# TonyLianLong/LLM-groundedDiffusion

Hardware: AMD Instinct MI355X
Metric: images/sec (50-step SD1.5 512^2, LMD+ guidance) (higher is better)
Workload: dtype fp16; 1 GPU; LMD+ stage 2, 4 cached 2-box layouts/GPU/step (lmd_v0.1 cache), 50 DDIM steps, 512x512, sd14_gligen (SD1.4+GLIGEN architecture, seeded random weights), VAE decodes included; per-box masks = box masks; mask_refinement=box, layouts_per_gpu=4, num_inference_steps=50, parallelism=dp1, rccl_ranks=1, lanes_per_gpu=4, gemm_tuning=throughput

## Files before the change

### llm-groundeddiffusion_amd/build.py

```python
import hashlib
import os
import subprocess
import sys

HERE = os.path.dirname(os.path.abspath(__file__))
CSRC = os.path.join(HERE, "csrc")
OUT = os.path.join(HERE, "liblgd_hip.so")
STAMP = OUT + ".stamp"
SOURCES = ["gemm.hip", "norm.hip", "attn.hip", "attn_w4.hip", "attn_bwd.hip", "misc.hip", "energy.hip", "boxdiff.hip", "sam.hip", "options.hip", "detect.hip", "sam_tail.hip", "handoff.hip"]
FLAGS = ["--offload-arch=gfx950", "-O3", "-std=c++17", "-fPIC",
         "-Wno-unused-value"]
EXTRA_FLAGS = {"attn.hip": ["-mllvm", "-amdgpu-mfma-vgpr-form=1"],
               "attn_bwd.hip": ["-mllvm", "-amdgpu-mfma-vgpr-form=1"],
               "sam_tail.hip": ["-ffp-contract=off"],
               "handoff.hip": ["-ffp-contract=off"]}


def _digest():
    h = hashlib.sha256()
    files = [os.path.join(CSRC, f) for f in sorted(os.listdir(CSRC))]
    files.append(os.path.join(HERE, "..", "include", "lgd_hip.h"))
    for f in files:
        with open(f, "rb") as fh:
            h.update(fh.read())
    h.update(" ".join(FLAGS).encode())
    h.update(repr(sorted(EXTRA_FLAGS.items())).encode())
    return h.hexdigest()


def build(force=False, verbose=True):
    dig = _digest()
    if not force and os.path.exists(OUT) and os.path.exists(STAMP):
        if open(STAMP).read().strip() == dig:
            return OUT
    hipcc = os.environ.get("HIPCC", "/opt/rocm/bin/hipcc")
    objs = []
    procs = []
    os.makedirs(os.path.join(HERE, "build"), exist_ok=True)
    for s in SOURCES:
        o = os.path.join(HERE, "build", s.replace(".hip", ".o"))
        cmd = [hipcc] + FLAGS + EXTRA_FLAGS.get(s, []) + ["-c", os.path.join(CSRC, s), "-o", o]
        procs.append((s, subprocess.Popen(cmd, stdout=subprocess.PIPE, stderr=subprocess.STDOUT)))
        objs.append(o)
    for s, p in procs:
        out, _ = p.communicate()
        if p.returncode != 0:
            raise RuntimeError(f"hipcc failed on {s}:\n{out.decode()}")
        if verbose and out.strip():
            print(out.decode())
    cmd = [hipcc, "--offload-arch=gfx950", "-shared", "-fPIC", "-o", OUT] + objs
    r = subprocess.run(cmd, stdout=subprocess.PIPE, stderr=subprocess.STDOUT)
    if r.returncode != 0:
        raise RuntimeError(f"link failed:\n{r.stdout.decode()}")
    with open(STAMP, "w") as fh:
        fh.write(dig)
    if verbose:
        print(f"built {OUT}")
    return OUT


if __name__ == "__main__":
    build(force="--force" in sys.argv)
```

### llm-groundeddiffusion_amd/csrc/attn_bwd.hip

```cpp
#include "common.h"
#include "../../include/lgd_hip.h"
#include "attn_plan.h"
#include <stdlib.h>

namespace {

constexpr int T64 = 64;
constexpr int TR_LD = T64 + 8;

template <int DP, int NT = 256>
struct PairTile {
  static constexpr int KSEG = DP / 8;
  static constexpr int ITEMS = (T64 / 2) * KSEG;
  static constexpr int IT = (ITEMS + NT - 1) / NT;
  uint4 v[IT][2];

  __device__ __forceinline__ void load(const half_t* __restrict__ src, long ld, int row0, int nrows, int d) {
#pragma unroll
    for (int i = 0; i < IT; ++i) {
      const int idx = threadIdx.x + i * NT;
      const int pair = idx & 31, seg = idx >> 5;
#pragma unroll
      for (int r = 0; r < 2; ++r) {
        const int row = row0 + pair * 2 + r;
        const bool ok = idx < ITEMS && row < nrows && seg * 8 < d;
        v[i][r] = ok ? *reinterpret_cast<const uint4*>(src + (long)row * ld + seg * 8) : make_uint4(0, 0, 0, 0);
      }
    }
  }
  template <bool RM, bool TR>
  __device__ __forceinline__ void store(half_t* rm, half_t* tr) const {
#pragma unroll
    for (int i = 0; i < IT; ++i) {
      const int idx = threadIdx.x + i * NT;
      if (idx >= ITEMS) continue;
      const int pair = idx & 31, seg = idx >> 5;
      if (RM) {
        *reinterpret_cast<uint4*>(rm + (pair * 2) * (DP + 16) + seg * 8) = v[i][0];
        *reinterpret_cast<uint4*>(rm + (pair * 2 + 1) * (DP + 16) + seg * 8) = v[i][1];
      }
      if (TR) {
        const uint32_t w0[4] = {v[i][0].x, v[i][0].y, v[i][0].z, v[i][0].w};
        const uint32_t w1[4] = {v[i][1].x, v[i][1].y, v[i][1].z, v[i][1].w};
#pragma unroll
        for (int j = 0; j < 4; ++j) {
          const uint32_t even = (w0[j] & 0xffffu) | (w1[j] << 16);
          const uint32_t odd = (w0[j] >> 16) | (w1[j] & 0xffff0000u);
          *reinterpret_cast<uint32_t*>(tr + (seg * 8 + 2 * j) * TR_LD + pair * 2) = even;
          *reinterpret_cast<uint32_t*>(tr + (seg * 8 + 2 * j + 1) * TR_LD + pair * 2) = odd;
        }
      }
    }
  }
};

struct AttnBwdArgs {
  const half_t* q; long ldq, q_bs;
  const half_t* k; long ldk, k_bs;
  const half_t* v; long ldv, v_bs;
  const half_t* o; long ldo, o_bs;
  const half_t* go; long ldgo, go_bs;
  const float* lse;
  float* delta;
  half_t* gq; long ldgq, gq_bs;
  half_t* gk; long ldgk, gk_bs;
  half_t* gv; long ldgv, gv_bs;
  int B, H, Sq, Sk, d;
  int sk_grad;
  float scale, scale_log2;
};

__device__ __forceinline__ half8_t tr_frag(const half_t* tr, int row, int c, int g) {
  const half_t* p = tr + row * TR_LD + c * 32 + g * 4;
  half4_t lo = *reinterpret_cast<const half4_t*>(p);
  half4_t hi = *reinterpret_cast<const half4_t*>(p + 16);
  return (half8_t){lo[0], lo[1], lo[2], lo[3], hi[0], hi[1], hi[2], hi[3]};
}

template <int DP, int QT, int NDT, int NW = 4, bool DB = false>
__global__ __launch_bounds__(64 * NW) void attn_bwd_dq_kernel(const AttnBwdArgs a) {
  constexpr int K_LD = DP + 16;
  constexpr int NDC = DP / 32;
  constexpr int STAGE = 2 * T64 * K_LD + DP * TR_LD;
  extern __shared__ __attribute__((aligned(16))) char dyn_smem[];
  half_t* const smem = reinterpret_cast<half_t*>(dyn_smem);
  half_t* Ks = smem;
  half_t* Vs = Ks + T64 * K_LD;
  half_t* Kt = Vs + T64 * K_LD;

  const int tid = threadIdx.x, lane = tid & 63, wid = tid >> 6;
  const int g = lane >> 4, c16 = lane & 15;
  const int b = blockIdx.z, h = blockIdx.y;
  const int d = a.d;
  const int q0 = blockIdx.x * (16 * NW * QT) + wid * (16 * QT);
  const half_t* Qb = a.q + (long)b * a.q_bs + (long)h * d;
  const half_t* Kb = a.k + (long)b * a.k_bs + (long)h * d;
  const half_t* Vb = a.v + (long)b * a.v_bs + (long)h * d;
  const half_t* Ob = a.o + (long)b * a.o_bs + (long)h * d;
  const half_t* GOb = a.go + (long)b * a.go_bs + (long)h * d;

  half8_t qf[QT][NDC], dof[QT][NDC];
  float delta[QT], nlse[QT];
#pragma unroll
  for (int qt = 0; qt < QT; ++qt) {
    const int qrow = q0 + qt * 16 + c16;
    const bool q_ok = qrow < a.Sq;
    float dl = 0.f;
#pragma unroll
    for (int dc = 0; dc < NDC; ++dc) {
      const int dd = dc * 32 + g * 8;
      if (q_ok && dd < d) {
        qf[qt][dc] = *reinterpret_cast<const half8_t*>(Qb + (long)qrow * a.ldq + dd);
        dof[qt][dc] = *reinterpret_cast<const half8_t*>(GOb + (long)qrow * a.ldgo + dd);
        half8_t of = *reinterpret_cast<const half8_t*>(Ob + (long)qrow * a.ldo + dd);
#pragma unroll
        for (int e = 0; e < 8; ++e) dl += (float)dof[qt][dc][e] * (float)of[e];
      } else {
        qf[qt][dc] = (half8_t){0, 0, 0, 0, 0, 0, 0, 0};
        dof[qt][dc] = (half8_t){0, 0, 0, 0, 0, 0, 0, 0};
      }
    }
    dl += __shfl_xor(dl, 16, 64);
    dl += __shfl_xor(dl, 32, 64);
    const long stat_idx = ((long)b * a.H + h) * a.Sq + qrow;
    if (q_ok && g == 0) a.delta[stat_idx] = dl;
    delta[qt] = dl;
    nlse[qt] = q_ok ? -a.lse[stat_idx] : 0.f;
  }

  f32x4 dq[QT][NDT];
#pragma unroll
  for (int qt = 0; qt < QT; ++qt)
#pragma unroll
    for (int dt = 0; dt < NDT; ++dt) dq[qt][dt] = (f32x4){0.f, 0.f, 0.f, 0.f};

  const float sl2 = a.scale_log2;
  const int n_tiles = (a.Sk + T64 - 1) / T64;
  PairTile<DP, 64 * NW> kreg, vreg;
  kreg.load(Kb, a.ldk, 0, a.Sk, d);
  vreg.load(Vb, a.ldv, 0, a.Sk, d);
  kreg.template store<true, true>(Ks, Kt);
  vreg.template store<true, false>(Vs, nullptr);
  __syncthreads();
  for (int t = 0; t < n_tiles; ++t) {
    const int kv0 = t * T64;
    if constexpr (DB) {
      Ks = smem + (t & 1) * STAGE;
      Vs = Ks + T64 * K_LD;
      Kt = Vs + T64 * K_LD;
    }
    if (t + 1 < n_tiles) {
      kreg.load(Kb, a.ldk, kv0 + T64, a.Sk, d);
      vreg.load(Vb, a.ldv, kv0 + T64, a.Sk, d);
    }
    f32x4 ds[QT][4];
#pragma unroll
    for (int kt = 0; kt < 4; ++kt) {
      half8_t kf[NDC], vf[NDC];
#pragma unroll
      for (int dc = 0; dc < NDC; ++dc) {
        kf[dc] = *reinterpret_cast<const half8_t*>(Ks + (kt * 16 + c16) * K_LD + dc * 32 + g * 8);
        vf[dc] = *reinterpret_cast<const half8_t*>(Vs + (kt * 16 + c16) * K_LD + dc * 32 + g * 8);
      }
#pragma unroll
      for (int qt = 0; qt < QT; ++qt) {
        f32x4 sv = {0.f, 0.f, 0.f, 0.f}, dp = {0.f, 0.f, 0.f, 0.f};
#pragma unroll
        for (int dc = 0; dc < NDC; ++dc) {
          sv = __builtin_amdgcn_mfma_f32_16x16x32_f16(kf[dc], qf[qt][dc], sv, 0, 0, 0);
          dp = __builtin_amdgcn_mfma_f32_16x16x32_f16(vf[dc], dof[qt][dc], dp, 0, 0, 0);
        }
#pragma unroll
        for (int r = 0; r < 4; ++r) {
          const float pv = __builtin_amdgcn_exp2f(fmaf(sv[r], sl2, nlse[qt]));
          ds[qt][kt][r] = pv * (dp[r] - delta[qt]);
        }
      }
    }
    if (kv0 + T64 > a.Sk) {
#pragma unroll
      for (int qt = 0; qt < QT; ++qt)
#pragma unroll
        for (int kt = 0; kt < 4; ++kt)
#pragma unroll
          for (int r = 0; r < 4; ++r)
            if (kv0 + kt * 16 + g * 4 + r >= a.Sk) ds[qt][kt][r] = 0.f;
    }
#pragma unroll
    for (int c = 0; c < 2; ++c) {
      half8_t dsf[QT];
#pragma unroll
      for (int qt = 0; qt < QT; ++qt)
#pragma unroll
        for (int r = 0; r < 4; ++r) {
          dsf[qt][r] = (half_t)ds[qt][2 * c][r];
          dsf[qt][4 + r] = (half_t)ds[qt][2 * c + 1][r];
        }
#pragma unroll
      for (int dt = 0; dt < NDT; ++dt) {
        half8_t ktf = tr_frag(Kt, dt * 16 + c16, c, g);
#pragma unroll
        for (int qt = 0; qt < QT; ++qt)
          dq[qt][dt] = __builtin_amdgcn_mfma_f32_16x16x32_f16(ktf, dsf[qt], dq[qt][dt], 0, 0, 0);
      }
    }
    if constexpr (DB) {
      if (t + 1 < n_tiles) {
        half_t* nK = smem + ((t + 1) & 1) * STAGE;
        kreg.template store<true, true>(nK, nK + 2 * T64 * K_LD);
        vreg.template store<true, false>(nK + T64 * K_LD, nullptr);
      }
      __syncthreads();
    } else {
      __syncthreads();
      if (t + 1 < n_tiles) {
        kreg.template store<true, true>(Ks, Kt);
        vreg.template store<true, false>(Vs, nullptr);
        __syncthreads();
      }
    }
  }
#pragma unroll
// ... 319 lines not shown
  const half_t* Vb = a.v + (long)b * a.v_bs + (long)h * d;

  for (int idx = tid; idx < XM_KEYS * KSEG; idx += 256) {
    const int row = idx / KSEG, seg = idx - row * KSEG;
    const bool ok = row < Sk && seg * 8 < d;
    const uint4 kk = ok ? *reinterpret_cast<const uint4*>(Kb + (long)row * a.ldk + seg * 8) : make_uint4(0, 0, 0, 0);
    const uint4 vv = ok ? *reinterpret_cast<const uint4*>(Vb + (long)row * a.ldv + seg * 8) : make_uint4(0, 0, 0, 0);
    *reinterpret_cast<uint4*>(Ks + row * K_LD + seg * 8) = kk;
    *reinterpret_cast<uint4*>(Vs + row * K_LD + seg * 8) = vv;
    const half_t* e = reinterpret_cast<const half_t*>(&kk);
#pragma unroll
    for (int j = 0; j < 8; ++j) Kt[(seg * 8 + j) * XM_LD + row] = e[j];
  }
  __syncthreads();

  const float sl2 = a.scale * 1.4426950408889634f;
  const int q_blk = blockIdx.x * 256;
  for (int it = 0; it < 4; ++it) {
    const int qrow = q_blk + it * 64 + wid * 16 + c16;
    if (q_blk + it * 64 + wid * 16 >= a.Sq) break;
    const bool q_ok = qrow < a.Sq;
    half8_t qf[NDC], gof[NDC];
#pragma unroll
    for (int dc = 0; dc < NDC; ++dc) {
      const int dd = dc * 32 + g * 8;
      qf[dc] = (half8_t){0, 0, 0, 0, 0, 0, 0, 0};
      gof[dc] = qf[dc];
      if (q_ok && dd < d) {
        qf[dc] = *reinterpret_cast<const half8_t*>(a.q + (long)b * a.q_bs + (long)qrow * a.ldq + (long)h * d + dd);
        if (a.go)
          gof[dc] = *reinterpret_cast<const half8_t*>(a.go + (long)b * a.go_bs + (long)qrow * a.ldgo + (long)h * d + dd);
      }
    }
    f32x4 sv[NKT], dp[NKT];
#pragma unroll
    for (int kt = 0; kt < NKT; ++kt) {
      f32x4 s = {0.f, 0.f, 0.f, 0.f}, t = {0.f, 0.f, 0.f, 0.f};
#pragma unroll
      for (int dc = 0; dc < NDC; ++dc) {
        half8_t kf = *reinterpret_cast<const half8_t*>(Ks + (kt * 16 + c16) * K_LD + dc * 32 + g * 8);
        half8_t vf = *reinterpret_cast<const half8_t*>(Vs + (kt * 16 + c16) * K_LD + dc * 32 + g * 8);
        s = __builtin_amdgcn_mfma_f32_16x16x32_f16(kf, qf[dc], s, 0, 0, 0);
        t = __builtin_amdgcn_mfma_f32_16x16x32_f16(vf, gof[dc], t, 0, 0, 0);
      }
      sv[kt] = s;
      dp[kt] = t;
    }
    float mx = -1.0e30f;
#pragma unroll
    for (int kt = 0; kt < NKT; ++kt)
#pragma unroll
      for (int r = 0; r < 4; ++r) {
        if (kt * 16 + g * 4 + r >= Sk) sv[kt][r] = -1.0e30f;
        mx = fmaxf(mx, sv[kt][r]);
      }
    mx = fmaxf(mx, __shfl_xor(mx, 16, 64));
    mx = fmaxf(mx, __shfl_xor(mx, 32, 64));
    const float nm = -mx * sl2;
    float sum = 0.f;
#pragma unroll
    for (int kt = 0; kt < NKT; ++kt)
#pragma unroll
      for (int r = 0; r < 4; ++r) {
        const float p = __builtin_amdgcn_exp2f(fmaf(sv[kt][r], sl2, nm));
        sv[kt][r] = p;
        sum += p;
      }
    sum += __shfl_xor(sum, 16, 64);
    sum += __shfl_xor(sum, 32, 64);
    const float inv = 1.f / sum;
    if (a.gp && q_ok) {
      const float* gpr = a.gp + (((long)b * a.H + h) * a.Sq + qrow) * Sk;
#pragma unroll
      for (int kt = 0; kt < NKT; ++kt)
#pragma unroll
        for (int r = 0; r < 4; ++r) {
          const int key = kt * 16 + g * 4 + r;
          if (key < Sk) dp[kt][r] += gpr[key];
        }
    }
    float dot = 0.f;
#pragma unroll
    for (int kt = 0; kt < NKT; ++kt)
#pragma unroll
      for (int r = 0; r < 4; ++r) {
        sv[kt][r] *= inv;
        dot += sv[kt][r] * dp[kt][r];
      }
    dot += __shfl_xor(dot, 16, 64);
    dot += __shfl_xor(dot, 32, 64);
    f32x4 dq[NDT];
#pragma unroll
    for (int dt = 0; dt < NDT; ++dt) dq[dt] = (f32x4){0.f, 0.f, 0.f, 0.f};
#pragma unroll
    for (int c = 0; c < NKT / 2; ++c) {
      half8_t dsf;
#pragma unroll
      for (int r = 0; r < 4; ++r) {
        dsf[r] = (half_t)(sv[2 * c][r] * (dp[2 * c][r] - dot) * a.scale);
        dsf[4 + r] = (half_t)(sv[2 * c + 1][r] * (dp[2 * c + 1][r] - dot) * a.scale);
      }
#pragma unroll
      for (int dt = 0; dt < NDT; ++dt) {
        const half_t* pk = Kt + (dt * 16 + c16) * XM_LD + c * 32 + g * 4;
        half4_t lo = *reinterpret_cast<const half4_t*>(pk);
        half4_t hi = *reinterpret_cast<const half4_t*>(pk + 16);
        half8_t ktf = {lo[0], lo[1], lo[2], lo[3], hi[0], hi[1], hi[2], hi[3]};
        dq[dt] = __builtin_amdgcn_mfma_f32_16x16x32_f16(ktf, dsf, dq[dt], 0, 0, 0);
      }
    }
    if (q_ok) {
      half_t* out = a.gq + (long)b * a.gq_bs + (long)qrow * a.ldgq + (long)h * d;
#pragma unroll
      for (int dt = 0; dt < NDT; ++dt) {
        const int dv = dt * 16 + g * 4;
        if (dv < d) {
          half4_t o;
#pragma unroll
          for (int r = 0; r < 4; ++r) o[r] = (half_t)dq[dt][r];
          *reinterpret_cast<half4_t*>(out + dv) = o;
        }
      }
    }
  }
}

template <int DP>
int launch_cross_bwd_mfma(const CrossBwdArgs& a, hipStream_t st) {
  const size_t smem = (size_t)(2 * XM_KEYS * (DP + 16) + DP * XM_LD) * 2;
  static const bool attr_set = [smem] {
    (void)hipFuncSetAttribute(reinterpret_cast<const void*>(&cross_attn_bwd_mfma_kernel<DP>),
                              hipFuncAttributeMaxDynamicSharedMemorySize, (int)smem);
    return true;
  }();
  (void)attr_set;
  hipLaunchKernelGGL((cross_attn_bwd_mfma_kernel<DP>), dim3((a.Sq + 255) / 256, a.H, a.B), dim3(256), smem, st, a);
  return lgd_check_launch();
}

int launch_cross_bwd_rows(const CrossBwdArgs& a, hipStream_t st) {
  const int ld = a.d + 2;
  size_t smem = (size_t)(2 * a.Sk * ld + 2) * 2 + (size_t)4 * 2 * XB_MAXD * 4 + (size_t)4 * XB_MAXSK * 4;
  smem = (smem + 15) & ~(size_t)15;
  static const bool attr_set = [] {
    (void)hipFuncSetAttribute(reinterpret_cast<const void*>(&cross_attn_bwd_kernel),
                        hipFuncAttributeMaxDynamicSharedMemorySize, 160 * 1024);
    return true;
  }();
  (void)attr_set;
  hipLaunchKernelGGL(cross_attn_bwd_kernel, dim3((a.Sq + 4 * XB_ROWS - 1) / (4 * XB_ROWS), a.H, a.B), dim3(256), smem, st, a);
  return lgd_check_launch();
}

template <int DP, int THREE, int SHAPE>
int launch_bwd(const AttnBwdArgs& a, hipStream_t st) {
  static_assert(!THREE || DP == 64, "the three-tile form is the d = 40 head at DP = 64");
  constexpr int NT = SHAPE == BWD_T1 ? 1 : 2, NDT = THREE ? 3 : DP / 16, NW = SHAPE == BWD_T2_DB_NW8 ? 8 : 4;
  constexpr bool DB = SHAPE == BWD_T2_DB || SHAPE == BWD_T2_DB_NW8;
  constexpr int K_LD = DP + 16;
  constexpr int NST = DB ? 2 : 1;
  const size_t smem_dq = (size_t)NST * (2 * T64 * K_LD + DP * TR_LD) * 2;
  const size_t smem_dkv = (size_t)NST * ((2 * T64 * K_LD + 2 * DP * TR_LD) * 2 + 2 * T64 * 4);
  static const bool attr_set = [smem_dq, smem_dkv] {
    (void)hipFuncSetAttribute(reinterpret_cast<const void*>(&attn_bwd_dkv_kernel<DP, NT, NDT, NW, DB>),
                        hipFuncAttributeMaxDynamicSharedMemorySize, (int)smem_dkv);
    (void)hipFuncSetAttribute(reinterpret_cast<const void*>(&attn_bwd_dq_kernel<DP, NT, NDT, NW, DB>),
                        hipFuncAttributeMaxDynamicSharedMemorySize, (int)smem_dq);
    return true;
  }();
  (void)attr_set;
  hipLaunchKernelGGL((attn_bwd_dq_kernel<DP, NT, NDT, NW, DB>), dim3((a.Sq + 16 * NW * NT - 1) / (16 * NW * NT), a.H, a.B),
                     dim3(64 * NW), smem_dq, st, a);
  hipLaunchKernelGGL((attn_bwd_dkv_kernel<DP, NT, NDT, NW, DB>), dim3((a.sk_grad + 16 * NW * NT - 1) / (16 * NW * NT), a.H, a.B),
                     dim3(64 * NW), smem_dkv, st, a);
  return lgd_check_launch();
}

int attn_bwd_env() {
  static const int env = [] { const char* e = getenv("LGD_ATTN_BWD"); return e ? atoi(e) : -2; }();
  return env;
}

int bwd_dp_of(int d) { return d <= 32 ? 32 : d <= 64 ? 64 : d <= 96 ? 96 : d <= 128 ? 128 : d <= 160 ? 160 : 0; }

int plan_bwd(int B, int H, int Sq, int Sk, int d) {
  const int DP = bwd_dp_of(d);
  if (!DP) return LGD_ERR_UNSUPPORTED;
  const long wgs = (long)((Sq < Sk ? Sq : Sk) / 128) * H * B;
  const int env = attn_bwd_env();
  const bool narrow = env == -2;
  const int mode = narrow ? 0 : env;
  if (DP == 64 && d <= 48) {
    if (wgs < 512) return attn_code(ATTN_FAM_BWD, DP, 10 + BWD_T1);
    if ((narrow || mode == 2) && wgs >= 1024) return attn_code(ATTN_FAM_BWD, DP, 10 + BWD_T2_DB_NW8);
    if (narrow || mode >= 1) return attn_code(ATTN_FAM_BWD, DP, 10 + BWD_T2_DB);
    return attn_code(ATTN_FAM_BWD, DP, 10 + BWD_T2);
  }
  if (DP <= 96 && wgs >= 512) {
    if (DP == 64 && mode == 2 && wgs >= 1024) return attn_code(ATTN_FAM_BWD, DP, BWD_T2_DB_NW8);
    if (mode >= 1) return attn_code(ATTN_FAM_BWD, DP, BWD_T2_DB);
    return attn_code(ATTN_FAM_BWD, DP, BWD_T2);
  }
  return attn_code(ATTN_FAM_BWD, DP, BWD_T1);
}

int plan_cross_bwd(int Sk, int d, bool aligned) {
  if (Sk < 1 || Sk > XB_MAXSK || d > XB_MAXD) return LGD_ERR_ARG;
  if (Sk <= XM_KEYS && d <= 160 && aligned) return attn_code(ATTN_FAM_XBWD_MFMA, bwd_dp_of(d), 0);
  return attn_code(ATTN_FAM_XBWD_ROWS, 0, 0);
}

#define BWD_NAME_T1 "1 tile per wave"
#define BWD_NAME_T2 "2 tiles per wave"
#define BWD_NAME_T2_DB "2 tiles per wave, double-buffered"
#define BWD_NAME_T2_DB_NW8 "2 tiles per wave, double-buffered, 8 waves"
#define BWD_NAME_THREE_0 " "
#define BWD_NAME_THREE_1 " (d <= 48, 3 tiles of d) "
#define BWD_ROW(DP, THREE, SHAPE, ENV)                                                                              \
  {{attn_code(ATTN_FAM_BWD, DP, 10 * THREE + BWD_##SHAPE), ENV,                                                     \
    "attn_bwd_dq/dkv_kernel DP=" #DP BWD_NAME_THREE_##THREE BWD_NAME_##SHAPE},                                      \
   launch_bwd<DP, THREE, BWD_##SHAPE>}
#define XBWD_MFMA_ROW(DP) {{attn_code(ATTN_FAM_XBWD_MFMA, DP, 0), 0, "cross_attn_bwd_mfma_kernel DP=" #DP}, launch_cross_bwd_mfma<DP>}

const AttnVariant<AttnBwdArgs> BWD_VARIANTS[] = {
    BWD_ROW(32, 0, T1, 0), BWD_ROW(32, 0, T2, 0), BWD_ROW(32, 0, T2_DB, 1),
    BWD_ROW(64, 0, T1, 0), BWD_ROW(64, 0, T2, 0), BWD_ROW(64, 0, T2_DB, 1), BWD_ROW(64, 0, T2_DB_NW8, 1),
    BWD_ROW(64, 1, T1, 0), BWD_ROW(64, 1, T2, 1), BWD_ROW(64, 1, T2_DB, 0), BWD_ROW(64, 1, T2_DB_NW8, 0),
    BWD_ROW(96, 0, T1, 0), BWD_ROW(96, 0, T2, 0), BWD_ROW(96, 0, T2_DB, 1),
    BWD_ROW(128, 0, T1, 0), BWD_ROW(160, 0, T1, 0),
};
const AttnVariant<CrossBwdArgs> XBWD_VARIANTS[] = {
    XBWD_MFMA_ROW(32), XBWD_MFMA_ROW(64), XBWD_MFMA_ROW(96), XBWD_MFMA_ROW(128), XBWD_MFMA_ROW(160),
    {{attn_code(ATTN_FAM_XBWD_ROWS, 0, 0), 0, "cross_attn_bwd_kernel (one wave per query row)"}, launch_cross_bwd_rows},
};
constexpr int N_BWD_VARIANTS = sizeof(BWD_VARIANTS) / sizeof(BWD_VARIANTS[0]);
constexpr int N_XBWD_VARIANTS = sizeof(XBWD_VARIANTS) / sizeof(XBWD_VARIANTS[0]);
static_assert(N_BWD_VARIANTS == 16 && N_XBWD_VARIANTS == 5 + 1, "a kernel instantiation was added or dropped");

}

int lgd_attn_bwd_plan(int B, int H, int Sq, int Sk, int d) { return plan_bwd(B, H, Sq, Sk, d); }
int lgd_cross_attn_bwd_plan(int Sk, int d, int aligned) { return plan_cross_bwd(Sk, d, aligned != 0); }
const AttnVariantInfo* lgd_attn_bwd_variant_info(int index) {
  if (index < 0) return nullptr;
  if (index < N_BWD_VARIANTS) return &BWD_VARIANTS[index].info;
  index -= N_BWD_VARIANTS;
  return index < N_XBWD_VARIANTS ? &XBWD_VARIANTS[index].info : nullptr;
}

extern "C" int lgd_attn_bwd_keys_f16(const void* q, int64_t ldq, int64_t q_bs, const void* k,
                                     int64_t ldk, int64_t k_bs, const void* v, int64_t ldv, int64_t v_bs,
                                     const void* o, int64_t ldo, int64_t o_bs, const void* go,
                                     int64_t ldgo, int64_t go_bs, const float* lse, float* delta, void* gq,
                                     int64_t ldgq, int64_t gq_bs, void* gk, int64_t ldgk, int64_t gk_bs,
                                     void* gv, int64_t ldgv, int64_t gv_bs, int B, int H, int Sq, int Sk,
                                     int Sk_grad, int d, float scale, void* stream) {
  if (int e = check_problem(B, H, Sq, Sk, d)) return e;
  if (Sk_grad < 1 || Sk_grad > Sk || !lse || !delta) return LGD_ERR_ARG;
  if (!attn_vectors_ok(d, {{q, ldq, q_bs}, {k, ldk, k_bs}, {v, ldv, v_bs}, {o, ldo, o_bs}, {go, ldgo, go_bs}},
                       {{gq, ldgq, gq_bs}, {gk, ldgk, gk_bs}, {gv, ldgv, gv_bs}}))
    return LGD_ERR_ARG;
  const int code = plan_bwd(B, H, Sq, Sk, d);
  if (code < 0) return code;
  (void)hipGetLastError();
  AttnBwdArgs a;
  a.q = (const half_t*)q; a.ldq = ldq; a.q_bs = q_bs;
  a.k = (const half_t*)k; a.ldk = ldk; a.k_bs = k_bs;
  a.v = (const half_t*)v; a.ldv = ldv; a.v_bs = v_bs;
  a.o = (const half_t*)o; a.ldo = ldo; a.o_bs = o_bs;
  a.go = (const half_t*)go; a.ldgo = ldgo; a.go_bs = go_bs;
  a.lse = lse; a.delta = delta;
  a.gq = (half_t*)gq; a.ldgq = ldgq; a.gq_bs = gq_bs;
  a.gk = (half_t*)gk; a.ldgk = ldgk; a.gk_bs = gk_bs;
  a.gv = (half_t*)gv; a.ldgv = ldgv; a.gv_bs = gv_bs;
  a.B = B; a.H = H; a.Sq = Sq; a.Sk = Sk; a.d = d;
  a.sk_grad = Sk_grad;
  a.scale = scale;
  a.scale_log2 = scale * 1.4426950408889634f;
  return attn_launch_code(BWD_VARIANTS, code, a, reinterpret_cast<hipStream_t>(stream));
}

extern "C" int lgd_attn_bwd_f16(const void* q, int64_t ldq, int64_t q_bs, const void* k,
                                int64_t ldk, int64_t k_bs, const void* v, int64_t ldv, int64_t v_bs,
                                const void* o, int64_t ldo, int64_t o_bs, const void* go,
                                int64_t ldgo, int64_t go_bs, const float* lse, float* delta, void* gq,
                                int64_t ldgq, int64_t gq_bs, void* gk, int64_t ldgk, int64_t gk_bs,
                                void* gv, int64_t ldgv, int64_t gv_bs, int B, int H, int Sq, int Sk,
                                int d, float scale, void* stream) {
  return lgd_attn_bwd_keys_f16(q, ldq, q_bs, k, ldk, k_bs, v, ldv, v_bs, o, ldo, o_bs, go, ldgo, go_bs, lse, delta, gq, ldgq,
                               gq_bs, gk, ldgk, gk_bs, gv, ldgv, gv_bs, B, H, Sq, Sk, Sk, d, scale, stream);
}

extern "C" int lgd_cross_attn_bwd_f16(const void* q, int64_t ldq, int64_t q_bs, const void* k,
                                      int64_t ldk, int64_t k_bs, const void* v, int64_t ldv,
                                      int64_t v_bs, const void* go, int64_t ldgo, int64_t go_bs,
                                      const float* gp, void* gq, int64_t ldgq, int64_t gq_bs, int B,
                                      int H, int Sq, int Sk, int d, float scale, void* stream) {
  if (check_problem(B, H, Sq, Sk, d) || Sk > XB_MAXSK || d > XB_MAXD || !gq ||
      !attn_vectors_ok(d, {{k, ldk, k_bs}, {v, ldv, v_bs}}, {}))
    return LGD_ERR_ARG;
  const AttnView Q{q, ldq, q_bs}, GO{go, ldgo, go_bs}, GQ{gq, ldgq, gq_bs};
  const bool aligned = Q.reads16() && GQ.writes8() && (ldgo % 8) == 0 && (!go || GO.reads16());
  const int code = plan_cross_bwd(Sk, d, aligned);
  if (code < 0) return code;
  (void)hipGetLastError();
  CrossBwdArgs a;
  a.q = (const half_t*)q; a.ldq = ldq; a.q_bs = q_bs;
  a.k = (const half_t*)k; a.ldk = ldk; a.k_bs = k_bs;
  a.v = (const half_t*)v; a.ldv = ldv; a.v_bs = v_bs;
// ... 7 lines not shown
```

Baseline: 1.816 images/s.

## Add hand-scheduled d=40 flash-attention backward kernels with AGPR accumulators and LDS DMA

Result: no change. 1.828 images/s (median of 6 runs) (+0.7%).

```diff
diff --git a/llm-groundeddiffusion_amd/build.py b/llm-groundeddiffusion_amd/build.py
--- a/llm-groundeddiffusion_amd/build.py
+++ b/llm-groundeddiffusion_amd/build.py
@@ -7,11 +7,12 @@
 CSRC = os.path.join(HERE, "csrc")
 OUT = os.path.join(HERE, "liblgd_hip.so")
 STAMP = OUT + ".stamp"
-SOURCES = ["gemm.hip", "norm.hip", "attn.hip", "attn_w4.hip", "attn_bwd.hip", "misc.hip", "energy.hip", "boxdiff.hip", "sam.hip", "options.hip", "detect.hip", "sam_tail.hip", "handoff.hip"]
+SOURCES = ["gemm.hip", "norm.hip", "attn.hip", "attn_w4.hip", "attn_bwd.hip", "attn_bwd_w4.hip", "misc.hip", "energy.hip", "boxdiff.hip", "sam.hip", "options.hip", "detect.hip", "sam_tail.hip", "handoff.hip"]
 FLAGS = ["--offload-arch=gfx950", "-O3", "-std=c++17", "-fPIC",
          "-Wno-unused-value"]
 EXTRA_FLAGS = {"attn.hip": ["-mllvm", "-amdgpu-mfma-vgpr-form=1"],
                "attn_bwd.hip": ["-mllvm", "-amdgpu-mfma-vgpr-form=1"],
+               "attn_bwd_w4.hip": ["-mllvm", "-amdgpu-mfma-vgpr-form=1"],
                "sam_tail.hip": ["-ffp-contract=off"],
                "handoff.hip": ["-ffp-contract=off"]}
 
diff --git a/llm-groundeddiffusion_amd/csrc/attn_bwd.hip b/llm-groundeddiffusion_amd/csrc/attn_bwd.hip
--- a/llm-groundeddiffusion_amd/csrc/attn_bwd.hip
+++ b/llm-groundeddiffusion_amd/csrc/attn_bwd.hip
@@ -1,6 +1,7 @@
 #include "common.h"
 #include "../../include/lgd_hip.h"
 #include "attn_plan.h"
+#include "attn_bwd_w4.h"
 #include <stdlib.h>
 
 namespace {
@@ -52,22 +53,6 @@
       }
     }
   }
-};
-
-struct AttnBwdArgs {
-  const half_t* q; long ldq, q_bs;
-  const half_t* k; long ldk, k_bs;
-  const half_t* v; long ldv, v_bs;
-  const half_t* o; long ldo, o_bs;
-  const half_t* go; long ldgo, go_bs;
-  const float* lse;
-  float* delta;
-  half_t* gq; long ldgq, gq_bs;
-  half_t* gk; long ldgk, gk_bs;
-  half_t* gv; long ldgv, gv_bs;
-  int B, H, Sq, Sk, d;
-  int sk_grad;
-  float scale, scale_log2;
 };
 
 __device__ __forceinline__ half8_t tr_frag(const half_t* tr, int row, int c, int g) {
@@ -693,9 +678,17 @@
   return lgd_check_launch();
 }
 
+bool bwd_w4_serves(const AttnBwdArgs& a, bool db_row) {
+  static const int env = [] { const char* e = getenv("LGD_ATTN_BWD_W4"); return e ? atoi(e) : 1; }();
+  if (env == 0 || a.d != 40) return false;
+  return env == 2 || db_row;
+}
+
 template <int DP, int THREE, int SHAPE>
 int launch_bwd(const AttnBwdArgs& a, hipStream_t st) {
   static_assert(!THREE || DP == 64, "the three-tile form is the d = 40 head at DP = 64");
+  if constexpr (THREE)
+    if (bwd_w4_serves(a, SHAPE == BWD_T2_DB || SHAPE == BWD_T2_DB_NW8)) return lgd_attn_bwd_w4_launch(a, st);
   constexpr int NT = SHAPE == BWD_T1 ? 1 : 2, NDT = THREE ? 3 : DP / 16, NW = SHAPE == BWD_T2_DB_NW8 ? 8 : 4;
   constexpr bool DB = SHAPE == BWD_T2_DB || SHAPE == BWD_T2_DB_NW8;
   constexpr int K_LD = DP + 16;
diff --git a/llm-groundeddiffusion_amd/csrc/attn_bwd_w4.h b/llm-groundeddiffusion_amd/csrc/attn_bwd_w4.h
--- /dev/null
+++ b/llm-groundeddiffusion_amd/csrc/attn_bwd_w4.h
@@ -0,0 +1,20 @@
+#pragma once
+#include "common.h"
+
+struct AttnBwdArgs {
+  const half_t* q; long ldq, q_bs;
+  const half_t* k; long ldk, k_bs;
+  const half_t* v; long ldv, v_bs;
+  const half_t* o; long ldo, o_bs;
+  const half_t* go; long ldgo, go_bs;
+  const float* lse;
+  float* delta;
+  half_t* gq; long ldgq, gq_bs;
+  half_t* gk; long ldgk, gk_bs;
+  half_t* gv; long ldgv, gv_bs;
+  int B, H, Sq, Sk, d;
+  int sk_grad;
+  float scale, scale_log2;
+};
+
+int lgd_attn_bwd_w4_launch(const AttnBwdArgs& a, hipStream_t st);
diff --git a/llm-groundeddiffusion_amd/csrc/attn_bwd_w4.hip b/llm-groundeddiffusion_amd/csrc/attn_bwd_w4.hip
--- /dev/null
+++ b/llm-groundeddiffusion_amd/csrc/attn_bwd_w4.hip
@@ -0,0 +1,409 @@
+#include "common.h"
+#include "attn_bwd_w4.h"
+#include <stdint.h>
+#include <type_traits>
+#include <utility>
+
+namespace {
+
+typedef short short4_t __attribute__((ext_vector_type(4)));
+typedef short short8_t __attribute__((ext_vector_type(8)));
+typedef __attribute__((address_space(3))) short4_t* lds_s4_ptr;
+
+__device__ __attribute__((aligned(64))) const half_t g_bw4_zeros[32] = {0, 0, 0, 0, 0, 0, 0, 0, 0, 0, 0, 0, 0, 0, 0, 0,
+                                                                        0, 0, 0, 0, 0, 0, 0, 0, 0, 0, 0, 0, 0, 0, 0, 0};
+
+constexpr int D = 40;
+constexpr int ROWB = 112;
+constexpr int SEGS = 7;
+constexpr int TILE_B = 64 * ROWB;
+constexpr int DQ_STAGE_B = 2 * TILE_B;
+constexpr int DQ_DUMMY_B = 2 * DQ_STAGE_B;
+constexpr int DQ_LDS_B = DQ_DUMMY_B + 1024 + 256;
+constexpr int KV_STAT_B = 2 * TILE_B;
+constexpr int KV_STAGE_B = KV_STAT_B + 512;
+constexpr int KV_LDS_B = 2 * KV_STAGE_B + 256;
+static_assert(KV_STAGE_B % 16 == 0 && TILE_B % 1024 == 0, "stages keep the alignment of the fragment reads");
+
+#define LGD_BW4_A10(t) "a" #t "0", "a" #t "1", "a" #t "2", "a" #t "3", "a" #t "4", "a" #t "5", "a" #t "6", "a" #t "7", "a" #t "8", "a" #t "9"
+#define LGD_BW4_AGPR_0_63 LGD_BW4_A10(), LGD_BW4_A10(1), LGD_BW4_A10(2), LGD_BW4_A10(3), LGD_BW4_A10(4), LGD_BW4_A10(5), "a60", "a61", "a62", "a63"
+#define LGD_BW4_AGPR_64_127                                                                                          \
+  "a64", "a65", "a66", "a67", "a68", "a69", LGD_BW4_A10(7), LGD_BW4_A10(8), LGD_BW4_A10(9), LGD_BW4_A10(10),         \
+  LGD_BW4_A10(11), "a120", "a121", "a122", "a123", "a124", "a125", "a126", "a127"
+
+template <int R0>
+__device__ __forceinline__ void mfma_acc(const half8_t& af, const half8_t& bf) {
+  asm volatile("s_nop 1\n\tv_mfma_f32_32x32x16_f16 a[%2:%3], %0, %1, a[%2:%3]" ::"v"(af), "v"(bf), "n"(R0), "n"(R0 + 15));
+}
+template <int R>
+__device__ __forceinline__ void agpr_write(float v) { asm volatile("v_accvgpr_write_b32 a[%1], %0" ::"v"(v), "n"(R)); }
+template <int R>
+__device__ __forceinline__ float agpr_read() { float v; asm volatile("v_accvgpr_read_b32 %0, a[%1]" : "=v"(v) : "n"(R)); return v; }
+template <int R0, int N>
+__device__ __forceinline__ void agpr_fill(float v) {
+  if constexpr (N > 0) { agpr_write<R0>(v); agpr_fill<R0 + 1, N - 1>(v); }
+}
+template <int R0>
+__device__ __forceinline__ half4_t agpr_half4(float mul) {
+  return (half4_t){(half_t)(agpr_read<R0>() * mul), (half_t)(agpr_read<R0 + 1>() * mul), (half_t)(agpr_read<R0 + 2>() * mul),
+                   (half_t)(agpr_read<R0 + 3>() * mul)};
+}
+template <int R0>
+__device__ __forceinline__ void store_row40(half_t* row, int hh, float mul, bool ok) {
+  const half4_t o0 = agpr_half4<R0 + 0>(mul), o1 = agpr_half4<R0 + 4>(mul), o2 = agpr_half4<R0 + 8>(mul),
+                o3 = agpr_half4<R0 + 12>(mul), o4 = agpr_half4<R0 + 16>(mul);
+  if (ok) {
+    *reinterpret_cast<half4_t*>(row + 0 + hh * 4) = o0;
+    *reinterpret_cast<half4_t*>(row + 8 + hh * 4) = o1;
+    *reinterpret_cast<half4_t*>(row + 16 + hh * 4) = o2;
+    *reinterpret_cast<half4_t*>(row + 24 + hh * 4) = o3;
+    *reinterpret_cast<half4_t*>(row + 32 + hh * 4) = o4;
+  }
+}
+
+__device__ __forceinline__ void dma16(const void* gptr, unsigned lds_addr) {
+  asm volatile("s_mov_b32 m0, %1\n\ts_nop 0\n\tglobal_load_lds_dwordx4 %0, off" ::"v"(gptr), "s"(__builtin_amdgcn_readfirstlane(lds_addr)) : "memory");
+}
+__device__ __forceinline__ void dma4(const void* gptr, unsigned lds_addr) {
+  asm volatile("s_mov_b32 m0, %1\n\ts_nop 0\n\tglobal_load_lds_dword %0, off" ::"v"(gptr), "s"(__builtin_amdgcn_readfirstlane(lds_addr)) : "memory");
+}
+
+__device__ __forceinline__ half8_t read_tr(const unsigned char* tr_lane, int row0, int cb) {
+  const unsigned char* p = tr_lane + row0 * ROWB + cb * 64;
+  const short4_t lo = __builtin_amdgcn_ds_read_tr16_b64_v4i16((lds_s4_ptr)(uintptr_t)(unsigned)(uintptr_t)p);
+  const short4_t hi = __builtin_amdgcn_ds_read_tr16_b64_v4i16((lds_s4_ptr)(uintptr_t)(unsigned)(uintptr_t)(p + 8 * ROWB));
+  const short8_t both = __builtin_shufflevector(lo, hi, 0, 1, 2, 3, 4, 5, 6, 7);
+  return __builtin_bit_cast(half8_t, both);
+}
+
+__device__ __forceinline__ half8_t load_frag(const half_t* row, int dd, bool ok) {
+  if (ok && dd < D) return *reinterpret_cast<const half8_t*>(row + dd);
+  return (half8_t){0, 0, 0, 0, 0, 0, 0, 0};
+}
+
+using I0 = std::integral_constant<int, 0>;
+using I1 = std::integral_constant<int, 1>;
+
+__global__ __launch_bounds__(256, 1) void attn_bwd_w4_dq_kernel(const AttnBwdArgs a) {
+  __shared__ __attribute__((aligned(1024))) unsigned char smem[DQ_LDS_B];
+  const int tid = threadIdx.x, lane = tid & 63;
+  const int wid = __builtin_amdgcn_readfirstlane(tid >> 6);
+  const int qi = lane & 31, hh = lane >> 5;
+  const int b = blockIdx.z, h = blockIdx.y;
+  const int q0 = blockIdx.x * 256 + wid * 64;
+  const half_t* Qb = a.q + (long)b * a.q_bs + (long)h * D;
+  const half_t* Kb = a.k + (long)b * a.k_bs + (long)h * D;
+  const half_t* Vb = a.v + (long)b * a.v_bs + (long)h * D;
+  const half_t* Ob = a.o + (long)b * a.o_bs + (long)h * D;
+  const half_t* GOb = a.go + (long)b * a.go_bs + (long)h * D;
+  const int n_tiles = (a.Sk + 63) >> 6;
+  const unsigned lds0 = (unsigned)(uintptr_t)smem;
+
+  for (int i = tid; i < DQ_LDS_B / 16; i += 256) reinterpret_cast<uint4*>(smem)[i] = make_uint4(0, 0, 0, 0);
+  __syncthreads();
+
+  asm volatile("" ::: LGD_BW4_AGPR_0_63);
+  {
+    float z;
+    asm volatile("v_mov_b32 %0, 0" : "=v"(z));
+    agpr_fill<0, 64>(z);
+    asm volatile("s_nop 15");
+  }
+
+  half8_t qf[2][3], gf[2][3];
+  float ndelta[2], nlse[2];
+#pragma unroll
+  for (int qb = 0; qb < 2; ++qb) {
+    const int qrow = q0 + qb * 32 + qi;
+    const bool q_ok = qrow < a.Sq;
+    float dl = 0.f;
+#pragma unroll
+    for (int ks = 0; ks < 3; ++ks) {
+      const int dd = ks * 16 + hh * 8;
+      qf[qb][ks] = load_frag(Qb + (long)qrow * a.ldq, dd, q_ok);
+      gf[qb][ks] = load_frag(GOb + (long)qrow * a.ldgo, dd, q_ok);
+      const half8_t of = load_frag(Ob + (long)qrow * a.ldo, dd, q_ok);
+#pragma unroll
+      for (int e = 0; e < 8; ++e) dl += (float)gf[qb][ks][e] * (float)of[e];
+    }
+    dl += __shfl_xor(dl, 32, 64);
+    const long stat_idx = ((long)b * a.H + h) * a.Sq + qrow;
+    if (q_ok && hh == 0) a.delta[stat_idx] = dl;
+    ndelta[qb] = -dl;
+    nlse[qb] = q_ok ? -a.lse[stat_idx] : 0.f;
+  }
+
+  const char* src[4];
+  long inc[4];
+  unsigned dst[4], smul[4];
+  int rr[2];
+  bool dat[2];
+#pragma unroll
+  for (int n = 0; n < 4; ++n) {
+    const bool isk = n >= 2;
+    const int j = wid + 4 * (n & 1);
+    const int x = j * 64 + lane;
+    const int r = x / SEGS, sg = x - r * SEGS;
+    const bool pad = j == 7;
+    rr[n & 1] = r;
+    dat[n & 1] = sg < 5 && !pad;
+    const long ld = isk ? a.ldk : a.ldv;
+    src[n] = reinterpret_cast<const char*>((isk ? Kb : Vb) + (long)r * ld + sg * 8);
+    inc[n] = 128 * ld;
+    dst[n] = lds0 + (pad ? DQ_DUMMY_B : (isk ? 0 : TILE_B) + j * 1024);
+    smul[n] = pad ? 0u : (unsigned)DQ_STAGE_B;
+  }
+  auto issue = [&](int t, unsigned stage) {
+#pragma unroll
+    for (int n = 0; n < 4; ++n) {
+      const bool ok = dat[n & 1] && t * 64 + rr[n & 1] < a.Sk;
+      dma16(ok ? src[n] : reinterpret_cast<const char*>(g_bw4_zeros), dst[n] + stage * smul[n]);
+      src[n] += inc[n];
+    }
+  };
+
+  const unsigned char* k_lane = smem + qi * ROWB + hh * 16;
+  const int j16 = lane & 15;
+  const unsigned char* tr_lane = smem + (4 * hh + (j16 >> 2)) * ROWB + (16 * ((lane >> 4) & 1) + 4 * (j16 & 3)) * 2;
+  const float sl2 = a.scale_log2;
+
+  auto half_tile = [&](int kb, unsigned stage, int key0, auto RAGGED) {
+    const unsigned char* kbase = k_lane + stage * DQ_STAGE_B + kb * 32 * ROWB;
+    half8_t kf[3], vf[3];
+#pragma unroll
+    for (int ks = 0; ks < 3; ++ks) {
+      kf[ks] = *reinterpret_cast<const half8_t*>(kbase + ks * 32);
+      vf[ks] = *reinterpret_cast<const half8_t*>(kbase + TILE_B + ks * 32);
+    }
+    float ds[2][16];
+#pragma unroll
+    for (int qb = 0; qb < 2; ++qb) {
+      f32x16 s = {0.f, 0.f, 0.f, 0.f, 0.f, 0.f, 0.f, 0.f, 0.f, 0.f, 0.f, 0.f, 0.f, 0.f, 0.f, 0.f};
+      f32x16 dp = s;
+#pragma unroll
+      for (int ks = 0; ks < 3; ++ks) {
+        s = __builtin_amdgcn_mfma_f32_32x32x16_f16(kf[ks], qf[qb][ks], s, 0, 0, 0);
+        dp = __builtin_amdgcn_mfma_f32_32x32x16_f16(vf[ks], gf[qb][ks], dp, 0, 0, 0);
+      }
+#pragma unroll
+      for (int i = 0; i < 16; ++i) {
+        const float pv = __builtin_amdgcn_exp2f(fmaf(s[i], sl2, nlse[qb]));
+        ds[qb][i] = pv * (dp[i] + ndelta[qb]);
+      }
+    }
+    if constexpr (decltype(RAGGED)::value) {
+#pragma unroll
+      for (int qb = 0; qb < 2; ++qb)
+#pragma unroll
+        for (int i = 0; i < 16; ++i)
+          if (key0 + 8 * (i >> 2) + 4 * hh + (i & 3) >= a.Sk) ds[qb][i] = 0.f;
+    }
+    half8_t dsf[2][2];
+#pragma unroll
+    for (int qb = 0; qb < 2; ++qb)
+#pragma unroll
+      for (int i = 0; i < 16; ++i) dsf[qb][i >> 3][i & 7] = (half_t)ds[qb][i];
+    const unsigned char* tbase = tr_lane + stage * DQ_STAGE_B;
+    {
+      const half8_t t00 = read_tr(tbase, kb * 32, 0), t01 = read_tr(tbase, kb * 32, 1);
+      const half8_t t10 = read_tr(tbase, kb * 32 + 16, 0), t11 = read_tr(tbase, kb * 32 + 16, 1);
+      mfma_acc<0>(t00, dsf[0][0]);  mfma_acc<32>(t00, dsf[1][0]);
+      mfma_acc<16>(t01, dsf[0][0]); mfma_acc<48>(t01, dsf[1][0]);
+      mfma_acc<0>(t10, dsf[0][1]);  mfma_acc<32>(t10, dsf[1][1]);
+      mfma_acc<16>(t11, dsf[0][1]); mfma_acc<48>(t11, dsf[1][1]);
+    }
+  };
+
+  issue(0, 0);
+  asm volatile("s_waitcnt vmcnt(0)" ::: "memory");
+  __syncthreads();
+  for (int t = 0; t < n_tiles; ++t) {
+    const unsigned stage = t & 1;
+    if (t + 1 < n_tiles) issue(t + 1, stage ^ 1);
+    if (t * 64 + 64 > a.Sk) {
+      half_tile(0, stage, t * 64, std::true_type{});
+      half_tile(1, stage, t * 64 + 32, std::true_type{});
+    } else {
+      half_tile(0, stage, t * 64, std::false_type{});
+      half_tile(1, stage, t * 64 + 32, std::false_type{});
+    }
+    asm volatile("s_waitcnt vmcnt(0) lgkmcnt(0)" ::: "memory");
+    __builtin_amdgcn_s_barrier();
+  }
+  asm volatile("s_nop 15\n\ts_nop 3");
+
+#pragma unroll
+  for (int qb = 0; qb < 2; ++qb) {
+    const int qrow = q0 + qb * 32 + qi;
+    half_t* out = a.gq + (long)b * a.gq_bs + (long)qrow * a.ldgq + (long)h * D;
+    if (qb == 0) store_row40<0>(out, hh, a.scale, qrow < a.Sq);
+    else store_row40<32>(out, hh, a.scale, qrow < a.Sq);
+  }
+}
+
+__global__ __launch_bounds__(256, 1) void attn_bwd_w4_dkv_kernel(const AttnBwdArgs a) {
+  __shared__ __attribute__((aligned(1024))) unsigned char smem[KV_LDS_B];
+  const int tid = threadIdx.x, lane = tid & 63;
+  const int wid = __builtin_amdgcn_readfirstlane(tid >> 6);
+  const int qi = lane & 31, hh = lane >> 5;
+  const int b = blockIdx.z, h = blockIdx.y;
+  const int k0 = blockIdx.x * 256 + wid * 64;
+  const half_t* Qb = a.q + (long)b * a.q_bs + (long)h * D;
+  const half_t* Kb = a.k + (long)b * a.k_bs + (long)h * D;
+  const half_t* Vb = a.v + (long)b * a.v_bs + (long)h * D;
+  const half_t* GOb = a.go + (long)b * a.go_bs + (long)h * D;
+  const float* lse_b = a.lse + ((long)b * a.H + h) * a.Sq;
+  const float* delta_b = a.delta + ((long)b * a.H + h) * a.Sq;
+  const int n_tiles = (a.Sq + 63) >> 6;
+  const unsigned lds0 = (unsigned)(uintptr_t)smem;
+
+  for (int i = tid; i < KV_LDS_B / 16; i += 256) reinterpret_cast<uint4*>(smem)[i] = make_uint4(0, 0, 0, 0);
+  __syncthreads();
+
+  asm volatile("" ::: LGD_BW4_AGPR_0_63, LGD_BW4_AGPR_64_127);
+  {
+    float z;
+    asm volatile("v_mov_b32 %0, 0" : "=v"(z));
+    agpr_fill<0, 128>(z);
+    asm volatile("s_nop 15");
+  }
+
+  half8_t kf[2][3], vf[2][3];
+#pragma unroll
+  for (int kb = 0; kb < 2; ++kb) {
+    const int krow = k0 + kb * 32 + qi;
+    const bool k_ok = krow < a.Sk;
+#pragma unroll
+    for (int ks = 0; ks < 3; ++ks) {
+      const int dd = ks * 16 + hh * 8;
+      kf[kb][ks] = load_frag(Kb + (long)krow * a.ldk, dd, k_ok);
+      vf[kb][ks] = load_frag(Vb + (long)krow * a.ldv, dd, k_ok);
+    }
+  }
+
+  const bool stat_wave = wid == 3;
+  const char* src[4];
+  long inc[4];
+  unsigned dst[4];
+  int rr[2];
+  bool dat[2];
+#pragma unroll
+  for (int n = 0; n < 4; ++n) {
+    const bool isg = n >= 2;
+    const int j = wid + 4 * (n & 1);
+    const int x = j * 64 + lane;
+    const int r = x / SEGS, sg = x - r * SEGS;
+    const long ld = isg ? a.ldgo : a.ldq;
+    if (j == 7) {
+      rr[1] = lane;
+      dat[1] = true;
+      src[n] = reinterpret_cast<const char*>((isg ? delta_b : lse_b) + lane);
+      inc[n] = 256;
+      dst[n] = lds0 + KV_STAT_B + (isg ? 256 : 0);
+    } else {
+      rr[n & 1] = r;
+      dat[n & 1] = sg < 5;
+      src[n] = reinterpret_cast<const char*>((isg ? GOb : Qb) + (long)r * ld + sg * 8);
+      inc[n] = 128 * ld;
+      dst[n] = lds0 + (isg ? TILE_B : 0) + j * 1024;
+    }
+  }
+  auto issue = [&](int t, unsigned stage) {
+#pragma unroll
+    for (int n = 0; n < 4; ++n) {
+      const bool ok = dat[n & 1] && t * 64 + rr[n & 1] < a.Sq;
+      const char* p = ok ? src[n] : reinterpret_cast<const char*>(g_bw4_zeros);
+      if ((n & 1) && stat_wave) dma4(p, dst[n] + stage * KV_STAGE_B);
+      else dma16(p, dst[n] + stage * KV_STAGE_B);
+      src[n] += inc[n];
+    }
+  };
+
+  const unsigned char* q_lane = smem + qi * ROWB + hh * 16;
+  const int j16 = lane & 15;
+  const unsigned char* tr_lane = smem + (4 * hh + (j16 >> 2)) * ROWB + (16 * ((lane >> 4) & 1) + 4 * (j16 & 3)) * 2;
+  const float sl2 = a.scale_log2;
+
+  auto half_tile = [&](int qh, unsigned stage) {
+    const unsigned char* sbase = smem + stage * KV_STAGE_B;
+    const unsigned char* qbase = q_lane + stage * KV_STAGE_B + qh * 32 * ROWB;
+    half8_t qa[3], ga[3];
+#pragma unroll
+    for (int ks = 0; ks < 3; ++ks) {
+      qa[ks] = *reinterpret_cast<const half8_t*>(qbase + ks * 32);
+      ga[ks] = *reinterpret_cast<const half8_t*>(qbase + TILE_B + ks * 32);
+    }
+    f32x4 ls[4], dl[4];
+#pragma unroll
+    for (int g4 = 0; g4 < 4; ++g4) {
+      ls[g4] = *reinterpret_cast<const f32x4*>(sbase + KV_STAT_B + (qh * 32 + 8 * g4 + 4 * hh) * 4);
+      dl[g4] = *reinterpret_cast<const f32x4*>(sbase + KV_STAT_B + 256 + (qh * 32 + 8 * g4 + 4 * hh) * 4);
+    }
+    half8_t pf[2][2], dsf[2][2];
+#pragma unroll
+    for (int kb = 0; kb < 2; ++kb) {
+      f32x16 s = {0.f, 0.f, 0.f, 0.f, 0.f, 0.f, 0.f, 0.f, 0.f, 0.f, 0.f, 0.f, 0.f, 0.f, 0.f, 0.f};
+      f32x16 dp = s;
+#pragma unroll
+      for (int ks = 0; ks < 3; ++ks) {
+        s = __builtin_amdgcn_mfma_f32_32x32x16_f16(qa[ks], kf[kb][ks], s, 0, 0, 0);
+        dp = __builtin_amdgcn_mfma_f32_32x32x16_f16(ga[ks], vf[kb][ks], dp, 0, 0, 0);
+      }
+#pragma unroll
+      for (int i = 0; i < 16; ++i) {
+        const float pv = __builtin_amdgcn_exp2f(fmaf(s[i], sl2, -ls[i >> 2][i & 3]));
+        pf[kb][i >> 3][i & 7] = (half_t)pv;
+        dsf[kb][i >> 3][i & 7] = (half_t)(pv * (dp[i] - dl[i >> 2][i & 3]));
+      }
+    }
+    const unsigned char* qt = tr_lane + stage * KV_STAGE_B;
+    const unsigned char* gt = qt + TILE_B;
+    {
+      const half8_t g00 = read_tr(gt, qh * 32, 0), g01 = read_tr(gt, qh * 32, 1);
+      const half8_t q00 = read_tr(qt, qh * 32, 0), q01 = read_tr(qt, qh * 32, 1);
+      mfma_acc<0>(g00, pf[0][0]);   mfma_acc<32>(g00, pf[1][0]);
+      mfma_acc<64>(q00, dsf[0][0]); mfma_acc<96>(q00, dsf[1][0]);
+      mfma_acc<16>(g01, pf[0][0]);  mfma_acc<48>(g01, pf[1][0]);
+      mfma_acc<80>(q01, dsf[0][0]); mfma_acc<112>(q01, dsf[1][0]);
+    }
+    {
+      const half8_t g10 = read_tr(gt, qh * 32 + 16, 0), g11 = read_tr(gt, qh * 32 + 16, 1);
+      const half8_t q10 = read_tr(qt, qh * 32 + 16, 0), q11 = read_tr(qt, qh * 32 + 16, 1);
+      mfma_acc<0>(g10, pf[0][1]);   mfma_acc<32>(g10, pf[1][1]);
+      mfma_acc<64>(q10, dsf[0][1]); mfma_acc<96>(q10, dsf[1][1]);
+      mfma_acc<16>(g11, pf[0][1]);  mfma_acc<48>(g11, pf[1][1]);
+      mfma_acc<80>(q11, dsf[0][1]); mfma_acc<112>(q11, dsf[1][1]);
+    }
+  };
+
+  issue(0, 0);
+  asm volatile("s_waitcnt vmcnt(0)" ::: "memory");
+  __syncthreads();
+  for (int t = 0; t < n_tiles; ++t) {
+    const unsigned stage = t & 1;
+    if (t + 1 < n_tiles) issue(t + 1, stage ^ 1);
+    half_tile(0, stage);
+    half_tile(1, stage);
+    asm volatile("s_waitcnt vmcnt(0) lgkmcnt(0)" ::: "memory");
+    __builtin_amdgcn_s_barrier();
+  }
+  asm volatile("s_nop 15\n\ts_nop 3");
+
+#pragma unroll
+  for (int kb = 0; kb < 2; ++kb) {
+    const int krow = k0 + kb * 32 + qi;
+    const bool ok = krow < a.sk_grad;
+    half_t* outk = a.gk + (long)b * a.gk_bs + (long)krow * a.ldgk + (long)h * D;
+    half_t* outv = a.gv + (long)b * a.gv_bs + (long)krow * a.ldgv + (long)h * D;
+    if (kb == 0) { store_row40<0>(outv, hh, 1.f, ok); store_row40<64>(outk, hh, a.scale, ok); }
+    else { store_row40<32>(outv, hh, 1.f, ok); store_row40<96>(outk, hh, a.scale, ok); }
+  }
+}
+
+}
+
+int lgd_attn_bwd_w4_launch(const AttnBwdArgs& a, hipStream_t st) {
+  hipLaunchKernelGGL(attn_bwd_w4_dq_kernel, dim3((a.Sq + 255) / 256, a.H, a.B), dim3(256), 0, st, a);
+  hipLaunchKernelGGL(attn_bwd_w4_dkv_kernel, dim3((a.sk_grad + 255) / 256, a.H, a.B), dim3(256), 0, st, a);
+  return lgd_check_launch();
+}
```
